# tasoc/photometry

Hardware: AMD Instinct MI355X
Metric: targets/sec (whole node), 10k targets x 1300 cad x 15x15, aperture + background (higher is better)
Workload: dtype f32

## Files before the change

### photometry_amd/csrc/aperture_dev.h

```cpp
#pragma once
#include "common.h"
#include <cmath>

namespace tp_ap {

constexpr int kMaxList = 128;
constexpr int kChunk = 1024;
constexpr int kMaxLeaves = 4096;
constexpr int kMaxDepth = 24;

template <int VEC> struct Vec;
template <> struct Vec<4> {
	static __device__ __forceinline__ void load(const float* p, float (&v)[4]) {
		float4 t = *reinterpret_cast<const float4*>(p);
		v[0] = t.x; v[1] = t.y; v[2] = t.z; v[3] = t.w;
	}
};
template <> struct Vec<2> {
	static __device__ __forceinline__ void load(const float* p, float (&v)[2]) {
		float2 t = *reinterpret_cast<const float2*>(p);
		v[0] = t.x; v[1] = t.y;
	}
};
template <> struct Vec<1> {
	static __device__ __forceinline__ void load(const float* p, float (&v)[1]) { v[0] = *p; }
};

template <int VEC>
struct CadState {
	float r[VEC][8];
	float e[VEC][8];
	float bk[VEC][8];
	float fres[VEC], eres[VEC], bres[VEC];
	double cw[VEC], ccol[VEC], crow[VEC];
	bool f_allnan[VEC], f_allzero[VEC], b_allnan[VEC];

	__device__ __forceinline__ void init() {
#pragma unroll
		for (int c = 0; c < VEC; c++) {
			fres[c] = 0.f; eres[c] = 0.f; bres[c] = 0.f;
			cw[c] = 0.0; ccol[c] = 0.0; crow[c] = 0.0;
			f_allnan[c] = true; f_allzero[c] = true; b_allnan[c] = true;
		}
	}
	__device__ __forceinline__ void side(const float (&v)[VEC], double col, double row) {
#pragma unroll
		for (int c = 0; c < VEC; c++) {
			const float x = v[c];
			f_allnan[c] = f_allnan[c] && (x != x);
			f_allzero[c] = f_allzero[c] && (x == 0.f);
			const double w = (x > 0.f) ? (double)x : 0.0;
			cw[c] += w;
			ccol[c] += col * w;
			crow[c] += row * w;
		}
	}
	__device__ __forceinline__ void bkg_terms(const float (&b)[VEC], float (&y)[VEC]) {
#pragma unroll
		for (int c = 0; c < VEC; c++) {
			const bool fin = (b[c] == b[c]);
			b_allnan[c] = b_allnan[c] && !fin;
			y[c] = fin ? b[c] : 0.f;
		}
	}
};

__device__ __forceinline__ float combine8(const float (&r)[8]) {
	return ((r[0] + r[1]) + (r[2] + r[3])) + ((r[4] + r[5]) + (r[6] + r[7]));
}

struct Args {
	const float* images; const float* images_err; const float* backgrounds;
	int32_t bkg_mode; int64_t bkg_series_pitch;
	const float* subtract; int64_t subtract_pitch;
	const uint8_t* mask; const int32_t* stamps; const int32_t* status;
	double* flux; double* flux_err; double* flux_bkg; double* ccol; double* crow;
	int64_t out_pitch; int n_cad; int height; int width; int64_t t_pitch; int n_targets;
	int32_t* big_list;
	int32_t stack_cols = 0, stack_row0 = 0, stack_col0 = 0;
};

__device__ __forceinline__ int64_t target_base(const Args& a, int target, int P) { return a.stack_cols ? 0 : (int64_t)target * P * a.t_pitch; }
__device__ __forceinline__ int stack_origin(const Args& a, int target) {
	return a.stack_cols ? ((a.stamps[target * 4 + 0] - a.stack_row0) * a.stack_cols + (a.stamps[target * 4 + 2] - a.stack_col0)) : 0;
}
__device__ __forceinline__ int pixel_row(const Args& a, int origin, int p, int pr, int pc) { return a.stack_cols ? (origin + pr * a.stack_cols + pc) : p; }

template <int VEC>
__device__ __forceinline__ void store_outputs(const Args& a, int target, int k0, const CadState<VEC>& st, int M) {
	const int64_t ob = (int64_t)target * a.out_pitch;
	const double nan = __builtin_nan("");
#pragma unroll
	for (int c = 0; c < VEC; c++) {
		const int k = k0 + c;
		if (k >= a.n_cad) continue;
		const bool bad = (M == 0) || st.f_allnan[c] || st.f_allzero[c];
		a.flux[ob + k] = bad ? nan : (double)st.fres[c];
		a.flux_err[ob + k] = bad ? nan : (double)sqrtf(st.eres[c]);
		const bool haspos = st.cw[c] > 0.0;
		a.ccol[ob + k] = (bad || !haspos) ? nan : st.ccol[c] / st.cw[c];
		a.crow[ob + k] = (bad || !haspos) ? nan : st.crow[c] / st.cw[c];
		if (a.flux_bkg) a.flux_bkg[ob + k] = (M == 0 || a.bkg_mode == 2 || st.b_allnan[c]) ? nan : (double)st.bres[c];
	}
}

__device__ __forceinline__ int compact_mask(const uint8_t* m, int P, int& p_next, int* list, int cap, int lane,
	bool count_rest, int* total)
{
	int n = 0;
	int p0 = p_next;
	for (; p0 < P; p0 += 64) {
		const int p = p0 + lane;
		const bool in = (p < P) && (m[p] != 0);
		const unsigned long long bal = __ballot(in);
		const int pos = n + __popcll(bal & ((1ull << lane) - 1ull));
		const int cnt = __popcll(bal);
		if (n + cnt > cap) {
			if (!count_rest) {
				if (in && pos < cap) list[pos] = p;
				const unsigned long long notstored = __ballot(in && pos >= cap);
				p_next = p0 + (int)__ffsll((long long)notstored) - 1;
				return cap;
			}
			if (in && pos < cap) list[pos] = p;
			n += cnt;
			continue;
		}
		if (in && pos < cap) list[pos] = p;
		n += cnt;
	}
	p_next = P;
	if (total) *total = n;
	return n < cap ? n : cap;
}

__device__ __forceinline__ void pack_rows(int* list, int M, int width, int lane, int nlanes) {
	for (int i = lane; i < M; i += nlanes) { const int p = list[i]; list[i] = p | ((p / width) << 16); }
}

template <int VEC>
__device__ __forceinline__ void extract_small(const Args& a, int target, const int* s_list, int M, int q_first, int q_stride)
{
	const int P = a.height * a.width;
	const int col0 = a.stamps[target * 4 + 2] + 1;
	const int row0 = a.stamps[target * 4 + 0] + 1;
	const int64_t tb = target_base(a, target, P);
	const int origin = stack_origin(a, target);
	const float* img = a.images + tb;
	const float* err = a.images_err + tb;
	const float* bkg = (a.bkg_mode == 0) ? (a.backgrounds + tb) : (a.backgrounds + (int64_t)target * a.bkg_series_pitch);
	const bool has_bkg = (a.bkg_mode != 2);
	const int nq = (a.n_cad + VEC - 1) / VEC;
	const int nblk = M - (M & 7);

	for (int q = q_first; q < nq; q += q_stride) {
		const int k0 = q * VEC;
		CadState<VEC> st;
		st.init();
		float bser[VEC], ssub[VEC];
		if (a.bkg_mode == 1) Vec<VEC>::load(bkg + k0, bser);
		if (a.subtract) Vec<VEC>::load(a.subtract + (int64_t)target * a.subtract_pitch + k0, ssub);

		auto fetch = [&](int idx, float (&v)[VEC], float (&e2)[VEC], float (&y)[VEC]) {
			const int pk = s_list[idx];
			const int p = pk & 0xffff;
			const int pr = (int)((unsigned)pk >> 16);
			const int pc = p - pr * a.width;
			const int64_t off = (int64_t)pixel_row(a, origin, p, pr, pc) * a.t_pitch + k0;
			float ee[VEC], bb[VEC];
			Vec<VEC>::load(img + off, v);
			if (a.subtract) {
#pragma unroll
				for (int c = 0; c < VEC; c++) v[c] = v[c] - ssub[c];
			}
			Vec<VEC>::load(err + off, ee);
			if (a.bkg_mode == 0) Vec<VEC>::load(bkg + off, bb);
			else {
#pragma unroll
				for (int c = 0; c < VEC; c++) bb[c] = (a.bkg_mode == 1) ? bser[c] : 0.f;
			}
#pragma unroll
			for (int c = 0; c < VEC; c++) e2[c] = ee[c] * ee[c];
			st.side(v, (double)(col0 + pc), (double)(row0 + pr));
			if (has_bkg) st.bkg_terms(bb, y);
		};

		if (M < 8) {
			for (int i = 0; i < M; i++) {
				float v[VEC], e2[VEC], y[VEC];
				fetch(i, v, e2, y);
#pragma unroll
				for (int c = 0; c < VEC; c++) { st.fres[c] += v[c]; st.eres[c] += e2[c]; if (has_bkg) st.bres[c] += y[c]; }
			}
		} else {
			for (int g = 0; g < nblk; g += 8) {
#pragma unroll
				for (int j = 0; j < 8; j++) {
					float v[VEC], e2[VEC], y[VEC];
					fetch(g + j, v, e2, y);
#pragma unroll
					for (int c = 0; c < VEC; c++) {
						if (g == 0) { st.r[c][j] = v[c]; st.e[c][j] = e2[c]; if (has_bkg) st.bk[c][j] = y[c]; }
						else { st.r[c][j] += v[c]; st.e[c][j] += e2[c]; if (has_bkg) st.bk[c][j] += y[c]; }
					}
				}
			}
#pragma unroll
			for (int c = 0; c < VEC; c++) { st.fres[c] = combine8(st.r[c]); st.eres[c] = combine8(st.e[c]); if (has_bkg) st.bres[c] = combine8(st.bk[c]); }
			for (int i = nblk; i < M; i++) {
				float v[VEC], e2[VEC], y[VEC];
				fetch(i, v, e2, y);
#pragma unroll
				for (int c = 0; c < VEC; c++) { st.fres[c] += v[c]; st.eres[c] += e2[c]; if (has_bkg) st.bres[c] += y[c]; }
			}
		}
#pragma unroll
		for (int c = 0; c < VEC; c++) { st.fres[c] = 0.f + st.fres[c]; st.eres[c] = 0.f + st.eres[c]; st.bres[c] = 0.f + st.bres[c]; }
		store_outputs<VEC>(a, target, k0, st, M);
	}
}

template <int VEC, bool HAS_SUB, int BKG, bool LDS_SERIES = false>
__device__ __forceinline__ void extract_small_stream(const Args& a, int target, const int* s_list, int M, int q_lane, int q_stride,
	const float* lds_sub = nullptr, const float* lds_ser = nullptr)
{
	const int P = a.height * a.width;
	const int col0 = a.stamps[target * 4 + 2] + 1;
	const int row0 = a.stamps[target * 4 + 0] + 1;
	const int64_t tb = (int64_t)target * P * a.t_pitch;
	const float* img = a.images + tb;
	const float* err = a.images_err + tb;
	constexpr bool BKG_CUBE = (BKG == 0), BKG_SERIES = (BKG == 1), HAS_BKG = (BKG != 2);
	const float* bkg = BKG_CUBE ? (a.backgrounds + tb) : (a.backgrounds + (int64_t)target * a.bkg_series_pitch);
	const float* subp = HAS_SUB ? (a.subtract + (int64_t)target * a.subtract_pitch) : nullptr;
	const int nq = (a.n_cad + VEC - 1) / VEC;
	const int nit = (nq + q_stride - 1) / q_stride;
	CadState<VEC> st;
	st.init();
	if (M == 0) {
		for (int it = 0; it < nit; it++) {
			const int q = q_lane + it * q_stride;
			if (q < nq) store_outputs<VEC>(a, target, q * VEC, st, 0);
		}
		return;
	}
	const int nfull = M >> 3, ntail = M & 7;
	const int spq = nfull + (ntail ? 1 : 0);
	const int total = nit * spq;

	struct Buf { float v[8][VEC], e[8][VEC], b[BKG_CUBE ? 8 : 1][VEC], ser[VEC], sub[VEC]; };
	Buf bufA, bufB;
	auto issue = [&](Buf& B, int step) {
		step = (step < total) ? step : (total - 1);
		const int it = step / spq, g = step - it * spq;
		int q = q_lane + it * q_stride;
		q = (q < nq) ? q : (nq - 1);
		const int k0 = q * VEC;
		if (BKG_SERIES) { if (LDS_SERIES) Vec<VEC>::load(lds_ser + k0, B.ser); else Vec<VEC>::load(bkg + k0, B.ser); }
		if (HAS_SUB) { if (LDS_SERIES) Vec<VEC>::load(lds_sub + k0, B.sub); else Vec<VEC>::load(subp + k0, B.sub); }
#pragma unroll
		for (int j = 0; j < 8; j++) {
			int idx = g * 8 + j;
			idx = (idx < M) ? idx : (M - 1);
			const int64_t rowoff = (int64_t)(__builtin_amdgcn_readfirstlane(s_list[idx]) & 0xffff) * a.t_pitch;
			Vec<VEC>::load(img + rowoff + k0, B.v[j]);
			Vec<VEC>::load(err + rowoff + k0, B.e[j]);
			if (BKG_CUBE) Vec<VEC>::load(bkg + rowoff + k0, B.b[j]);
		}
	};
	auto consume = [&](const Buf& B, int step) {
		if (step >= total) return;
		const int it = step / spq, g = step - it * spq;
		const int q = q_lane + it * q_stride;
		const bool full = g < nfull;
		const int cnt = full ? 8 : ntail;
#pragma unroll
		for (int j = 0; j < 8; j++) {
			if (j < cnt) {
				const int pk = __builtin_amdgcn_readfirstlane(s_list[g * 8 + j]);
				const int p = pk & 0xffff;
				const int pr = (int)((unsigned)pk >> 16);
				const int pc = p - pr * a.width;
				float v[VEC], e2[VEC], bb[VEC], y[VEC];
#pragma unroll
				for (int c = 0; c < VEC; c++) {
					v[c] = HAS_SUB ? (B.v[j][c] - B.sub[c]) : B.v[j][c];
					e2[c] = B.e[j][c] * B.e[j][c];
					bb[c] = BKG_CUBE ? B.b[BKG_CUBE ? j : 0][c] : (BKG_SERIES ? B.ser[c] : 0.f);
				}
				st.side(v, (double)(col0 + pc), (double)(row0 + pr));
				if (HAS_BKG) st.bkg_terms(bb, y);
#pragma unroll
				for (int c = 0; c < VEC; c++) {
					if (full) {
						if (g == 0) { st.r[c][j] = v[c]; st.e[c][j] = e2[c]; if (HAS_BKG) st.bk[c][j] = y[c]; }
						else { st.r[c][j] += v[c]; st.e[c][j] += e2[c]; if (HAS_BKG) st.bk[c][j] += y[c]; }
					} else { st.fres[c] += v[c]; st.eres[c] += e2[c]; if (HAS_BKG) st.bres[c] += y[c]; }
				}
			}
		}
		if (full && g == nfull - 1) {
#pragma unroll
			for (int c = 0; c < VEC; c++) { st.fres[c] = combine8(st.r[c]); st.eres[c] = combine8(st.e[c]); if (HAS_BKG) st.bres[c] = combine8(st.bk[c]); }
		}
		if (g == spq - 1) {
#pragma unroll
			for (int c = 0; c < VEC; c++) { st.fres[c] = 0.f + st.fres[c]; st.eres[c] = 0.f + st.eres[c]; st.bres[c] = 0.f + st.bres[c]; }
			if (q < nq) store_outputs<VEC>(a, target, q * VEC, st, M);
			st.init();
		}
	};
	issue(bufA, 0);
	issue(bufB, 1);
	for (int step = 0; step < total; step += 2) {
		consume(bufA, step);
		issue(bufA, step + 2);
		consume(bufB, step + 1);
		issue(bufB, step + 3);
	}
}

}

int tp_aperture_extract_big(tp_ctx* ctx, const tp_ap::Args& a, bool vec4);

void* tp_ctx_scratch(tp_ctx* ctx, size_t bytes);
```

### photometry_amd/csrc/fused.hip

```cpp
#include "sumimage_dev.h"
#include "aperture_dev.h"
#include "k2p2_args.h"
#include <algorithm>
#include <vector>

namespace {

constexpr int kRows = 8;

template <int VEC, bool VEC4, bool HAS_SUB, int BKG, bool A1>
__global__ __launch_bounds__(64, 2) void tp_aperture_fused_kernel(tp_ap::Args a, k2p2::BatchArgs ka, k2p2::Params prm,
	const double* __restrict__ twid, const int32_t* __restrict__ quality, int64_t quality_stride, uint32_t bitmask,
	double* __restrict__ sumimage_out, const int32_t* __restrict__ order)
{
	extern __shared__ __align__(16) unsigned char smem[];
	const int target = order ? order[blockIdx.x] : (int)blockIdx.x;
	const int lane = threadIdx.x;
	k2p2::Shared k;
	k2p2::shared_carve(k, smem, ka.H, ka.W, lane, twid);
	const int P = ka.H * ka.W;

	if constexpr (!A1) {
		const double* in = sumimage_out + (int64_t)target * P;
		for (int p = lane; p < P; p += 64) k.S[p] = in[p];
	} else {
	unsigned char* good = reinterpret_cast<unsigned char*>(k.srt);
	tp_sum::stage_good(good, quality + (int64_t)target * quality_stride, bitmask, a.n_cad, lane, 64);
	__syncthreads();
	{
		const float* base = a.images + (int64_t)target * P * a.t_pitch;
		const float* sub = a.subtract ? (a.subtract + (int64_t)target * a.subtract_pitch) : nullptr;
		double* o = sumimage_out + (int64_t)target * P;
		int p = 0;
		if (VEC4) {
			const int nq = ((a.n_cad + 3) & ~3) >> 2;
			const int spg = (nq + 63) >> 6;
			const int ngroups = (P + kRows - 1) / kRows;
			const uint32_t* good4 = reinterpret_cast<const uint32_t*>(good);
			const float4* sub4 = reinterpret_cast<const float4*>(sub);
			const float4 zero4 = make_float4(0.f, 0.f, 0.f, 0.f);
			const int total = ngroups * spg;
			float4 bufA[kRows], bufB[kRows];
			float4 subA = zero4, subB = zero4;
			auto issue = [&](float4 (&buf)[kRows], float4& sbuf, int st) {
				st = (st < total) ? st : (total - 1);
				const int g = st / spg, i = st - g * spg;
				int qd = lane + (i << 6);
				qd = (qd < nq) ? qd : (nq - 1);
				if (HAS_SUB) sbuf = sub4[qd];
#pragma unroll
				for (int j = 0; j < kRows; j++) {
					int r = g * kRows + j;
					r = (r < P) ? r : (P - 1);
					buf[j] = reinterpret_cast<const float4*>(base + (int64_t)r * a.t_pitch)[qd];
				}
			};
			double sacc[kRows];
			int nacc[kRows];
#pragma unroll
			for (int j = 0; j < kRows; j++) { sacc[j] = 0.0; nacc[j] = 0; }
			auto consume = [&](const float4 (&buf)[kRows], const float4& sa, int st) {
				const bool valid = st < total;
				const int g = st / spg, i = st - g * spg;
				const int qd = lane + (i << 6);
				if (valid && qd < nq) {
					const uint32_t gd = good4[qd];
#pragma unroll
					for (int j = 0; j < kRows; j++) {
						float4 v = buf[j];
						if (HAS_SUB) { v.x -= sa.x; v.y -= sa.y; v.z -= sa.z; v.w -= sa.w; }
						tp_sum::acc1(v.x, gd & 0xffu, sacc[j], nacc[j]); tp_sum::acc1(v.y, gd & 0xff00u, sacc[j], nacc[j]);
						tp_sum::acc1(v.z, gd & 0xff0000u, sacc[j], nacc[j]); tp_sum::acc1(v.w, gd & 0xff000000u, sacc[j], nacc[j]);
					}
				}
				if (valid && i == spg - 1) {
#pragma unroll
					for (int off = 32; off > 0; off >>= 1) {
#pragma unroll
						for (int j = 0; j < kRows; j++) { sacc[j] += __shfl_down(sacc[j], off, 64); nacc[j] += __shfl_down(nacc[j], off, 64); }
					}
					if (lane == 0) {
#pragma unroll
						for (int j = 0; j < kRows; j++) {
							const int r = g * kRows + j;
							if (r < P) { const double m = (nacc[j] > 0) ? sacc[j] / (double)nacc[j] : __builtin_nan(""); k.S[r] = m; o[r] = m; }
						}
					}
#pragma unroll
					for (int j = 0; j < kRows; j++) { sacc[j] = 0.0; nacc[j] = 0; }
				}
			};
			issue(bufA, subA, 0);
			issue(bufB, subB, 1);
			for (int st = 0; st < total; st += 2) {
				consume(bufA, subA, st);
				issue(bufA, subA, st + 2);
				consume(bufB, subB, st + 1);
				issue(bufB, subB, st + 3);
			}
		} else {
			for (; p < P; p++) {
				const double m = tp_sum::row_mean_scalar(base + (int64_t)p * a.t_pitch, sub, good, a.n_cad, lane);
				if (lane == 0) { k.S[p] = m; o[p] = m; }
			}
		}
	}
	}
	__syncthreads();

	k2p2::Target t;
	k2p2::make_target(ka, target, t);
	t.S = k.S;
	const int status = k2p2::run_target(k, prm, t);
	if (status == TP_STATUS_ERROR) return;

	int* s_list = reinterpret_cast<int*>(k.lab);
	int pn = 0, M = 0;
	tp_ap::compact_mask(k.res, P, pn, s_list, tp_ap::kMaxList, lane, true, &M);
	__syncthreads();
	if (M > tp_ap::kMaxList) {
		if (lane == 0 && a.big_list) a.big_list[1 + atomicAdd(&a.big_list[0], 1)] = target;
		return;
	}
	tp_ap::pack_rows(s_list, M, a.width, lane, 64);
	__syncthreads();
	const float* lds_sub = nullptr;
	const float* lds_ser = nullptr;
	{
		constexpr bool SER = (BKG == 1);
		const float* gsub = HAS_SUB ? (a.subtract + (int64_t)target * a.subtract_pitch) : nullptr;
		const float* gser = SER ? (a.backgrounds + (int64_t)target * a.bkg_series_pitch) : nullptr;
		const int nflt = (a.n_cad + VEC - 1) / VEC * VEC;
		const int room = (int)((reinterpret_cast<unsigned char*>(s_list) - smem) / sizeof(float));
		float* stage = reinterpret_cast<float*>(smem);
		const bool same = HAS_SUB && SER && (gsub == gser);
		const int need = ((HAS_SUB ? 1 : 0) + ((SER && !same) ? 1 : 0)) * nflt;
		if ((HAS_SUB || SER) && need > 0 && need <= room) {
			if (HAS_SUB) { for (int i = lane; i < nflt; i += 64) stage[i] = gsub[(i < a.n_cad) ? i : (a.n_cad - 1)]; lds_sub = stage; }
			if (SER) {
				if (same) lds_ser = stage;
				else { float* st2 = stage + (HAS_SUB ? nflt : 0); for (int i = lane; i < nflt; i += 64) st2[i] = gser[(i < a.n_cad) ? i : (a.n_cad - 1)]; lds_ser = st2; }
			}
			__syncthreads();
		}
	}
	if ((HAS_SUB && lds_sub) || (BKG == 1 && lds_ser)) tp_ap::extract_small_stream<VEC, HAS_SUB, BKG, true>(a, target, s_list, M, lane, 64, lds_sub, lds_ser);
	else tp_ap::extract_small_stream<VEC, HAS_SUB, BKG, false>(a, target, s_list, M, lane, 64);
}

}

static const int32_t* fused_launch_order(tp_ctx* ctx, const double* d_tmag, int n)
{
	if (n < 4096 || d_tmag == nullptr) return nullptr;
	if (ctx->order && ctx->order_key == (const void*)d_tmag && ctx->order_n == n) return ctx->order;
	std::vector<double> tm((size_t)n);
	if (hipMemcpyAsync(tm.data(), d_tmag, (size_t)n * sizeof(double), hipMemcpyDeviceToHost, ctx->stream) != hipSuccess) return nullptr;
	if (hipStreamSynchronize(ctx->stream) != hipSuccess) return nullptr;
	std::vector<int32_t> idx((size_t)n);
	for (int i = 0; i < n; ++i) idx[(size_t)i] = i;
	std::stable_sort(idx.begin(), idx.end(), [&](int32_t x, int32_t y) { return tm[(size_t)x] < tm[(size_t)y]; });
	if (ctx->order_n < n) {
		if (ctx->order) (void)hipFree(ctx->order);
		ctx->order = nullptr; ctx->order_n = 0;
		void* p = nullptr;
		if (tp_device_alloc(ctx, &p, (size_t)n * sizeof(int32_t)) != hipSuccess) return nullptr;
		ctx->order = static_cast<int32_t*>(p);
	}
	if (hipMemcpy(ctx->order, idx.data(), (size_t)n * sizeof(int32_t), hipMemcpyHostToDevice) != hipSuccess) { ctx->order_key = nullptr; return nullptr; }
	ctx->order_key = d_tmag; ctx->order_n = n;
	return ctx->order;
}

static int aperture_photometry_impl(tp_ctx* ctx, const tp_cube_desc* desc, bool given_sumimage,
	const float* d_images, const float* d_images_err, const float* d_backgrounds, int32_t bkg_mode, int64_t bkg_series_pitch,
	const float* d_subtract, int64_t subtract_pitch,
	const int32_t* d_quality, int64_t quality_target_stride, uint32_t bitmask,
	const int64_t* d_cat_offsets, const float* d_cat_column_stamp, const float* d_cat_row_stamp, const float* d_cat_tmag,
	const float* d_cat_column, const float* d_cat_row, const int64_t* d_cat_starid,
	const double* d_target_pos_row, const double* d_target_pos_column, const double* d_target_tmag, const int64_t* d_target_starid,
	const int32_t* d_stamps, const int32_t* d_aperture, const tp_k2p2_params* params,
	double* d_sumimage, uint8_t* d_mask, int32_t* d_status, int32_t* d_flags, double* d_contamination, double* d_diag,
	uint8_t* d_cat_in_mask,
	double* d_flux, double* d_flux_err, double* d_flux_background, double* d_centroid_col, double* d_centroid_row, int64_t out_pitch)
{
	TP_CHECK_CTX(ctx);
	TP_API_BEGIN
	TP_REQUIRE(ctx, tp_desc_ok(desc), "tp_aperture_photometry: bad cube descriptor");
	TP_REQUIRE(ctx, d_images && d_images_err && (d_quality || given_sumimage) && d_stamps && d_aperture && d_cat_offsets
		&& d_target_pos_row && d_target_pos_column && d_target_tmag && d_target_starid, "tp_aperture_photometry: null input pointer");
	TP_REQUIRE(ctx, d_sumimage && d_mask && d_status && d_flags && d_contamination, "tp_aperture_photometry: null output pointer");
	TP_REQUIRE(ctx, d_flux && d_flux_err && d_centroid_col && d_centroid_row, "tp_aperture_photometry: null output pointer");
	TP_REQUIRE(ctx, d_flux_background || !d_backgrounds, "tp_aperture_photometry: backgrounds given but no flux_background output");
	TP_REQUIRE(ctx, out_pitch >= desc->n_cad, "tp_aperture_photometry: out_pitch < n_cad");
	TP_REQUIRE(ctx, bkg_mode == 0 || bkg_mode == 1, "tp_aperture_photometry: bkg_mode must be 0 (cube) or 1 (series)");
	if (!d_backgrounds) bkg_mode = 2;
	TP_REQUIRE(ctx, bkg_mode != 1 || bkg_series_pitch >= desc->n_cad, "tp_aperture_photometry: bad bkg_series_pitch");
	TP_REQUIRE(ctx, quality_target_stride == 0 || quality_target_stride >= desc->n_cad, "tp_aperture_photometry: bad quality stride");
	TP_REQUIRE(ctx, d_subtract == nullptr || subtract_pitch >= desc->n_cad, "tp_aperture_photometry: bad subtract pitch");
	if (desc->n_targets == 0) return TP_OK;
	const int P = desc->height * desc->width;
	const k2p2::SharedLayout lay = k2p2::shared_layout(P);
	size_t shmem = lay.total;
	const size_t a1_bytes = lay.off_region + (size_t)((desc->n_cad + 3) & ~3) + 16;
	if (!given_sumimage && a1_bytes > shmem) shmem = a1_bytes;
	if (shmem > 160 * 1024) {
		int rc = given_sumimage ? TP_OK : tp_sumimage(ctx, desc, d_images, d_quality, quality_target_stride, bitmask, d_subtract, subtract_pitch, d_sumimage);
		if (rc != TP_OK) return rc;
		rc = tp_k2p2_masks(ctx, desc->n_targets, desc->height, desc->width, d_sumimage, d_cat_offsets, d_cat_column_stamp, d_cat_row_stamp,
			d_cat_tmag, d_cat_column, d_cat_row, d_cat_starid, d_target_pos_row, d_target_pos_column, d_target_tmag, d_target_starid,
			d_stamps, d_aperture, nullptr, params, d_mask, d_status, d_flags, d_contamination, d_diag, d_cat_in_mask);
		if (rc != TP_OK) return rc;
		return tp_aperture_extract(ctx, desc, d_images, d_images_err, d_backgrounds, (bkg_mode == 2) ? 0 : bkg_mode, bkg_series_pitch,
			d_subtract, subtract_pitch, d_mask, d_stamps, d_status, d_flux, d_flux_err, d_flux_background, d_centroid_col, d_centroid_row, out_pitch);
	}

	if (!ctx->twiddle) {
		double h[2 * k2p2::kGrid];
		for (int j = 0; j < k2p2::kGrid; ++j) {
			h[j] = std::cos(2.0 * k2p2::kPi * (double)j / (double)k2p2::kGrid);
			h[k2p2::kGrid + j] = std::sin(2.0 * k2p2::kPi * (double)j / (double)k2p2::kGrid);
		}
		TP_HIP(ctx, hipMalloc(&ctx->twiddle, sizeof(h)));
		TP_HIP(ctx, hipMemcpy(ctx->twiddle, h, sizeof(h), hipMemcpyHostToDevice));
	}

	k2p2::Params prm = k2p2::default_params();
	if (params) {
		prm.thresh = params->thresh;
		prm.min_no_pixels_in_mask = params->min_no_pixels_in_mask;
		prm.min_for_cluster = params->min_for_cluster;
		prm.extend_overflow = params->extend_overflow;
		prm.ws_thres = params->ws_thres;
		prm.saturation_limit = params->saturation_limit;
	}
	k2p2::BatchArgs ka;
	ka.n_targets = desc->n_targets; ka.H = desc->height; ka.W = desc->width; ka.sumimage = d_sumimage; ka.cat_offsets = d_cat_offsets;
	ka.cat_column_stamp = d_cat_column_stamp; ka.cat_row_stamp = d_cat_row_stamp; ka.cat_tmag = d_cat_tmag;
	ka.cat_column = d_cat_column; ka.cat_row = d_cat_row; ka.cat_starid = d_cat_starid;
	ka.target_pos_row = d_target_pos_row; ka.target_pos_column = d_target_pos_column; ka.target_tmag = d_target_tmag;
	ka.target_starid = d_target_starid; ka.stamps = d_stamps; ka.aperture = d_aperture; ka.cut_override = nullptr;
	ka.mask = d_mask; ka.status = d_status; ka.flags = d_flags; ka.contamination = d_contamination; ka.diag = d_diag;
	ka.cat_in_mask = d_cat_in_mask;

	tp_ap::Args a;
	a.images = d_images; a.images_err = d_images_err; a.backgrounds = d_backgrounds;
	a.bkg_mode = bkg_mode; a.bkg_series_pitch = bkg_series_pitch;
	a.subtract = d_subtract; a.subtract_pitch = subtract_pitch;
	a.mask = d_mask; a.stamps = d_stamps; a.status = d_status;
	a.flux = d_flux; a.flux_err = d_flux_err; a.flux_bkg = d_flux_background;
	a.ccol = d_centroid_col; a.crow = d_centroid_row;
	a.out_pitch = out_pitch; a.n_cad = desc->n_cad; a.height = desc->height; a.width = desc->width;
	a.t_pitch = desc->t_pitch; a.n_targets = desc->n_targets;
	a.big_list = static_cast<int32_t*>(tp_ctx_scratch(ctx, ((size_t)desc->n_targets + 1) * sizeof(int32_t)));
	TP_REQUIRE(ctx, a.big_list != nullptr, "tp_aperture_photometry: out of device memory for the work list");
	TP_HIP(ctx, hipMemsetAsync(a.big_list, 0, sizeof(int32_t), ctx->stream));

	bool vec4 = tp_vec4_ok(d_images, desc->t_pitch) && tp_vec4_ok(d_images_err, desc->t_pitch);
	if (bkg_mode == 0) vec4 = vec4 && tp_vec4_ok(d_backgrounds, desc->t_pitch);
	else if (bkg_mode == 1) vec4 = vec4 && tp_vec4_ok(d_backgrounds, bkg_series_pitch);
	if (d_subtract) vec4 = vec4 && tp_vec4_ok(d_subtract, subtract_pitch);

	const int32_t* d_order = fused_launch_order(ctx, d_target_tmag, desc->n_targets);
	const dim3 grid((unsigned)desc->n_targets), block(64);
#define TP_FUSED_LAUNCH_A(V, V4, HS, BK, A1) do { \
		auto kern = tp_aperture_fused_kernel<V, V4, HS, BK, A1>; \
		if (shmem > 64 * 1024) TP_HIP(ctx, hipFuncSetAttribute(reinterpret_cast<const void*>(kern), hipFuncAttributeMaxDynamicSharedMemorySize, (int)shmem)); \
		TP_LAUNCH(ctx, TPK_FUSED, kern, grid, block, shmem, a, ka, prm, (const double*)ctx->twiddle, d_quality, quality_target_stride, bitmask, d_sumimage, d_order); \
	} while (0)
#define TP_FUSED_LAUNCH(V, V4, HS, BK) do { if (given_sumimage) TP_FUSED_LAUNCH_A(V, V4, HS, BK, false); else TP_FUSED_LAUNCH_A(V, V4, HS, BK, true); } while (0)
#define TP_FUSED_BKG(V, V4, HS) do { \
		if (bkg_mode == 0) TP_FUSED_LAUNCH(V, V4, HS, 0); else if (bkg_mode == 1) TP_FUSED_LAUNCH(V, V4, HS, 1); else TP_FUSED_LAUNCH(V, V4, HS, 2); \
	} while (0)
	if (vec4) { if (d_subtract) TP_FUSED_BKG(2, true, true); else TP_FUSED_BKG(2, true, false); }
	else { if (d_subtract) TP_FUSED_BKG(1, false, true); else TP_FUSED_BKG(1, false, false); }
#undef TP_FUSED_BKG
#undef TP_FUSED_LAUNCH
#undef TP_FUSED_LAUNCH_A
	TP_LAUNCH_CHECK(ctx, "tp_aperture_fused_kernel");
	return tp_aperture_extract_big(ctx, a, vec4);
	TP_API_END(ctx)
}

extern "C" int tp_aperture_photometry(tp_ctx* ctx, const tp_cube_desc* desc,
	const float* d_images, const float* d_images_err, const float* d_backgrounds, int32_t bkg_mode, int64_t bkg_series_pitch,
	const float* d_subtract, int64_t subtract_pitch,
	const int32_t* d_quality, int64_t quality_target_stride, uint32_t bitmask,
	const int64_t* d_cat_offsets, const float* d_cat_column_stamp, const float* d_cat_row_stamp, const float* d_cat_tmag,
	const float* d_cat_column, const float* d_cat_row, const int64_t* d_cat_starid,
	const double* d_target_pos_row, const double* d_target_pos_column, const double* d_target_tmag, const int64_t* d_target_starid,
	const int32_t* d_stamps, const int32_t* d_aperture, const tp_k2p2_params* params,
	double* d_sumimage, uint8_t* d_mask, int32_t* d_status, int32_t* d_flags, double* d_contamination, double* d_diag,
	uint8_t* d_cat_in_mask,
	double* d_flux, double* d_flux_err, double* d_flux_background, double* d_centroid_col, double* d_centroid_row, int64_t out_pitch)
{
	return aperture_photometry_impl(ctx, desc, false, d_images, d_images_err, d_backgrounds, bkg_mode, bkg_series_pitch, d_subtract, subtract_pitch,
		d_quality, quality_target_stride, bitmask, d_cat_offsets, d_cat_column_stamp, d_cat_row_stamp, d_cat_tmag, d_cat_column, d_cat_row, d_cat_starid,
		d_target_pos_row, d_target_pos_column, d_target_tmag, d_target_starid, d_stamps, d_aperture, params, d_sumimage, d_mask, d_status, d_flags,
		d_contamination, d_diag, d_cat_in_mask, d_flux, d_flux_err, d_flux_background, d_centroid_col, d_centroid_row, out_pitch);
}

extern "C" int tp_aperture_photometry_from_sumimage(tp_ctx* ctx, const tp_cube_desc* desc,
	const float* d_images, const float* d_images_err, const float* d_backgrounds, int32_t bkg_mode, int64_t bkg_series_pitch,
	const float* d_subtract, int64_t subtract_pitch,
	const int32_t* d_quality, int64_t quality_target_stride, uint32_t bitmask,
	const int64_t* d_cat_offsets, const float* d_cat_column_stamp, const float* d_cat_row_stamp, const float* d_cat_tmag,
	const float* d_cat_column, const float* d_cat_row, const int64_t* d_cat_starid,
	const double* d_target_pos_row, const double* d_target_pos_column, const double* d_target_tmag, const int64_t* d_target_starid,
	const int32_t* d_stamps, const int32_t* d_aperture, const tp_k2p2_params* params,
	const double* d_sumimage, uint8_t* d_mask, int32_t* d_status, int32_t* d_flags, double* d_contamination, double* d_diag,
	uint8_t* d_cat_in_mask,
	double* d_flux, double* d_flux_err, double* d_flux_background, double* d_centroid_col, double* d_centroid_row, int64_t out_pitch)
{
	return aperture_photometry_impl(ctx, desc, true, d_images, d_images_err, d_backgrounds, bkg_mode, bkg_series_pitch, d_subtract, subtract_pitch,
		d_quality, quality_target_stride, bitmask, d_cat_offsets, d_cat_column_stamp, d_cat_row_stamp, d_cat_tmag, d_cat_column, d_cat_row, d_cat_starid,
		d_target_pos_row, d_target_pos_column, d_target_tmag, d_target_starid, d_stamps, d_aperture, params, const_cast<double*>(d_sumimage), d_mask, d_status, d_flags,
		d_contamination, d_diag, d_cat_in_mask, d_flux, d_flux_err, d_flux_background, d_centroid_col, d_centroid_row, out_pitch);
}
```

Before: 1.401 million.

## Precompute per-pixel offset and coordinate table in LDS for streaming aperture extraction

Builds a per-target LDS table of 32-bit byte offsets and double column/row coordinates, replacing per-pixel readfirstlane list decoding and 64-bit address math in the streaming loop. The step counters become incremental, which removes divisions. The accumulation is restructured with a new state struct that handles series backgrounds and optional FMA centroid accumulation. Launch bounds are raised to three waves per SIMD for most variants. It adds LDS usage, a fallback path when offsets overflow 32 bits, and may change rounding of centroid sums when FMA is used.

```diff
diff --git a/photometry_amd/csrc/aperture_dev.h b/photometry_amd/csrc/aperture_dev.h
--- a/photometry_amd/csrc/aperture_dev.h
+++ b/photometry_amd/csrc/aperture_dev.h
@@ -86,8 +86,8 @@
 }
 __device__ __forceinline__ int pixel_row(const Args& a, int origin, int p, int pr, int pc) { return a.stack_cols ? (origin + pr * a.stack_cols + pc) : p; }
 
-template <int VEC>
-__device__ __forceinline__ void store_outputs(const Args& a, int target, int k0, const CadState<VEC>& st, int M) {
+template <int VEC, class State>
+__device__ __forceinline__ void store_outputs(const Args& a, int target, int k0, const State& st, int M) {
 	const int64_t ob = (int64_t)target * a.out_pitch;
 	const double nan = __builtin_nan("");
 #pragma unroll
@@ -220,22 +220,78 @@
 	}
 }
 
-template <int VEC, bool HAS_SUB, int BKG, bool LDS_SERIES = false>
-__device__ __forceinline__ void extract_small_stream(const Args& a, int target, const int* s_list, int M, int q_lane, int q_stride,
+struct PixelTable { const double* col; const double* row; const uint32_t* off; };
+
+constexpr int kPixelEntryBytes = 20;
+__host__ __device__ inline int pixel_table_entries(int M) { return (M + 7) & ~7; }
+__host__ __device__ inline bool stream_offsets_fit(int64_t P, int64_t t_pitch) { return P * t_pitch * 4 < ((int64_t)1 << 32); }
+
+__device__ __forceinline__ PixelTable build_pixel_table(void* mem, const int* list, int M, const Args& a, int target, int lane, int nlanes)
+{
+	const int M8 = pixel_table_entries(M);
+	double* col = static_cast<double*>(mem);
+	double* row = col + M8;
+	uint32_t* off = reinterpret_cast<uint32_t*>(row + M8);
+	const int col0 = a.stamps[target * 4 + 2] + 1;
+	const int row0 = a.stamps[target * 4 + 0] + 1;
+	for (int i = lane; i < M8; i += nlanes) {
+		const int p = list[(i < M) ? i : (M - 1)];
+		const int pr = p / a.width, pc = p - pr * a.width;
+		off[i] = (uint32_t)p * (uint32_t)a.t_pitch * 4u;
+		col[i] = (double)(col0 + pc);
+		row[i] = (double)(row0 + pr);
+	}
+	PixelTable t;
+	t.col = col; t.row = row; t.off = off;
+	return t;
+}
+
+template <int VEC, int NBK>
+struct StreamState {
+	float r[VEC][8], e[VEC][8], bk[VEC][NBK];
+	float fres[VEC], eres[VEC], bres[VEC];
+	double cw[VEC], ccol[VEC], crow[VEC];
+	bool f_allnan[VEC], f_allzero[VEC], b_allnan[VEC];
+
+	__device__ __forceinline__ void init() {
+#pragma unroll
+		for (int c = 0; c < VEC; c++) {
+#pragma unroll
+			for (int j = 0; j < 8; j++) { r[c][j] = -0.f; e[c][j] = -0.f; }
+#pragma unroll
+			for (int j = 0; j < NBK; j++) bk[c][j] = -0.f;
+			fres[c] = 0.f; eres[c] = 0.f; bres[c] = 0.f;
+			cw[c] = 0.0; ccol[c] = 0.0; crow[c] = 0.0;
+			f_allnan[c] = true; f_allzero[c] = true; b_allnan[c] = true;
+		}
+	}
+	template <bool FUSE>
+	__device__ __forceinline__ void side(int c, float x, double col, double row) {
+		f_allnan[c] = f_allnan[c] && (x != x);
+		f_allzero[c] = f_allzero[c] && (x == 0.f);
+		const double w = (double)__builtin_fmaxf(x, 0.f);
+		cw[c] += w;
+		if (FUSE) { ccol[c] = __builtin_fma(col, w, ccol[c]); crow[c] = __builtin_fma(row, w, crow[c]); }
+		else { ccol[c] += col * w; crow[c] += row * w; }
+	}
+};
+
+#define TP_AP_KEEP_SCALAR(x) asm volatile("" : "+s"(x))
+template <int VEC, bool HAS_SUB, int BKG, bool LDS_SERIES, bool FUSE>
+__device__ __forceinline__ void extract_small_stream(const Args& a, int target, const PixelTable& tbl, int M, int q_lane, int q_stride,
 	const float* lds_sub = nullptr, const float* lds_ser = nullptr)
 {
 	const int P = a.height * a.width;
-	const int col0 = a.stamps[target * 4 + 2] + 1;
-	const int row0 = a.stamps[target * 4 + 0] + 1;
 	const int64_t tb = (int64_t)target * P * a.t_pitch;
-	const float* img = a.images + tb;
-	const float* err = a.images_err + tb;
 	constexpr bool BKG_CUBE = (BKG == 0), BKG_SERIES = (BKG == 1), HAS_BKG = (BKG != 2);
-	const float* bkg = BKG_CUBE ? (a.backgrounds + tb) : (a.backgrounds + (int64_t)target * a.bkg_series_pitch);
+	const char* img = reinterpret_cast<const char*>(a.images + tb);
+	const char* err = reinterpret_cast<const char*>(a.images_err + tb);
+	const char* bkgc = BKG_CUBE ? reinterpret_cast<const char*>(a.backgrounds + tb) : nullptr;
+	const float* bser = BKG_SERIES ? (a.backgrounds + (int64_t)target * a.bkg_series_pitch) : nullptr;
 	const float* subp = HAS_SUB ? (a.subtract + (int64_t)target * a.subtract_pitch) : nullptr;
 	const int nq = (a.n_cad + VEC - 1) / VEC;
 	const int nit = (nq + q_stride - 1) / q_stride;
-	CadState<VEC> st;
+	StreamState<VEC, BKG_CUBE ? 8 : 1> st;
 	st.init();
 	if (M == 0) {
 		for (int it = 0; it < nit; it++) {
@@ -246,79 +302,138 @@
 	}
 	const int nfull = M >> 3, ntail = M & 7;
 	const int spq = nfull + (ntail ? 1 : 0);
-	const int total = nit * spq;
 
 	struct Buf { float v[8][VEC], e[8][VEC], b[BKG_CUBE ? 8 : 1][VEC], ser[VEC], sub[VEC]; };
 	Buf bufA, bufB;
-	auto issue = [&](Buf& B, int step) {
-		step = (step < total) ? step : (total - 1);
-		const int it = step / spq, g = step - it * spq;
-		int q = q_lane + it * q_stride;
+	int it_i = 0, g_i = 0, it_c = 0, g_c = 0;
+	auto issue = [&](Buf& B) {
+		int q = q_lane + it_i * q_stride;
 		q = (q < nq) ? q : (nq - 1);
 		const int k0 = q * VEC;
-		if (BKG_SERIES) { if (LDS_SERIES) Vec<VEC>::load(lds_ser + k0, B.ser); else Vec<VEC>::load(bkg + k0, B.ser); }
-		if (HAS_SUB) { if (LDS_SERIES) Vec<VEC>::load(lds_sub + k0, B.sub); else Vec<VEC>::load(subp + k0, B.sub); }
+		if (!LDS_SERIES) {
+			if (BKG_SERIES) Vec<VEC>::load(bser + k0, B.ser);
+			if (HAS_SUB) Vec<VEC>::load(subp + k0, B.sub);
+		}
+		const uint4* to = reinterpret_cast<const uint4*>(tbl.off + g_i * 8);
+		const uint4 o0 = to[0], o1 = to[1];
+		const uint32_t ro[8] = { o0.x, o0.y, o0.z, o0.w, o1.x, o1.y, o1.z, o1.w };
+		const uint32_t kb = (uint32_t)k0 * 4u;
 #pragma unroll
 		for (int j = 0; j < 8; j++) {
-			int idx = g * 8 + j;
-			idx = (idx < M) ? idx : (M - 1);
-			const int64_t rowoff = (int64_t)(__builtin_amdgcn_readfirstlane(s_list[idx]) & 0xffff) * a.t_pitch;
-			Vec<VEC>::load(img + rowoff + k0, B.v[j]);
-			Vec<VEC>::load(err + rowoff + k0, B.e[j]);
-			if (BKG_CUBE) Vec<VEC>::load(bkg + rowoff + k0, B.b[j]);
-		}
+			const uint64_t vo = (uint64_t)(ro[j] + kb);
+			Vec<VEC>::load(reinterpret_cast<const float*>(img + vo), B.v[j]);
+			Vec<VEC>::load(reinterpret_cast<const float*>(err + vo), B.e[j]);
+			if (BKG_CUBE) Vec<VEC>::load(reinterpret_cast<const float*>(bkgc + vo), B.b[BKG_CUBE ? j : 0]);
+		}
+		if (++g_i == spq) { g_i = 0; ++it_i; }
+		if (it_i == nit) { it_i = nit - 1; g_i = spq - 1; }
 	};
-	auto consume = [&](const Buf& B, int step) {
-		if (step >= total) return;
-		const int it = step / spq, g = step - it * spq;
-		const int q = q_lane + it * q_stride;
-		const bool full = g < nfull;
-		const int cnt = full ? 8 : ntail;
-#pragma unroll
-		for (int j = 0; j < 8; j++) {
-			if (j < cnt) {
-				const int pk = __builtin_amdgcn_readfirstlane(s_list[g * 8 + j]);
-				const int p = pk & 0xffff;
-				const int pr = (int)((unsigned)pk >> 16);
-				const int pc = p - pr * a.width;
-				float v[VEC], e2[VEC], bb[VEC], y[VEC];
+	auto pixel = [&](const Buf& B, const float (&sub)[VEC], int j, double col, double row, float (&v)[VEC], float (&e2)[VEC], float (&y)[VEC]) {
+#pragma unroll
+		for (int c = 0; c < VEC; c++) {
+			v[c] = HAS_SUB ? (B.v[j][c] - sub[c]) : B.v[j][c];
+			e2[c] = B.e[j][c] * B.e[j][c];
+			st.template side<FUSE>(c, v[c], col, row);
+			if (BKG_CUBE) {
+				const float b = B.b[BKG_CUBE ? j : 0][c];
+				const bool fin = (b == b);
+				st.b_allnan[c] = st.b_allnan[c] && !fin;
+				y[c] = fin ? b : 0.f;
+			}
+		}
+	};
+	auto consume = [&](const Buf& B) {
+		if (it_c == nit) return;
+		const int q = q_lane + it_c * q_stride;
+		float ser[VEC], sub[VEC], yser[VEC];
+#pragma unroll
+		for (int c = 0; c < VEC; c++) { ser[c] = B.ser[c]; sub[c] = B.sub[c]; }
+		if (LDS_SERIES) {
+			const int k0 = ((q < nq) ? q : (nq - 1)) * VEC;
+			if (BKG_SERIES) Vec<VEC>::load(lds_ser + k0, ser);
+			if (HAS_SUB) Vec<VEC>::load(lds_sub + k0, sub);
+		}
+		if (BKG_SERIES) {
+#pragma unroll
+			for (int c = 0; c < VEC; c++) { const bool fin = (ser[c] == ser[c]); st.b_allnan[c] = !fin; yser[c] = fin ? ser[c] : 0.f; }
+		}
+		constexpr int NP = (LDS_SERIES && !BKG_CUBE) ? 4 : 2;
+		const double2* tc = reinterpret_cast<const double2*>(tbl.col + g_c * 8);
+		const double2* tr = reinterpret_cast<const double2*>(tbl.row + g_c * 8);
+		if (g_c < nfull) {
+#pragma unroll
+			for (int h = 0; h < 8 / NP; h++) {
+				if (h) __builtin_amdgcn_sched_barrier(0);
+				double col[NP], row[NP];
+#pragma unroll
+				for (int i = 0; i < NP / 2; i++) {
+					const double2 cc = tc[h * (NP / 2) + i], rr = tr[h * (NP / 2) + i];
+					col[2 * i] = cc.x; col[2 * i + 1] = cc.y; row[2 * i] = rr.x; row[2 * i + 1] = rr.y;
+				}
+#pragma unroll
+				for (int jj = 0; jj < NP; jj++) {
+					const int j = NP * h + jj;
+					float v[VEC], e2[VEC], y[VEC];
+					pixel(B, sub, j, col[jj], row[jj], v, e2, y);
+#pragma unroll
+					for (int c = 0; c < VEC; c++) { st.r[c][j] += v[c]; st.e[c][j] += e2[c]; if (BKG_CUBE) st.bk[c][BKG_CUBE ? j : 0] += y[c]; }
+				}
+			}
+			if (BKG_SERIES) {
+#pragma unroll
+				for (int c = 0; c < VEC; c++) st.bk[c][0] += yser[c];
+			}
+			if (g_c == nfull - 1) {
 #pragma unroll
 				for (int c = 0; c < VEC; c++) {
-					v[c] = HAS_SUB ? (B.v[j][c] - B.sub[c]) : B.v[j][c];
-					e2[c] = B.e[j][c] * B.e[j][c];
-					bb[c] = BKG_CUBE ? B.b[BKG_CUBE ? j : 0][c] : (BKG_SERIES ? B.ser[c] : 0.f);
+					st.r[c][0] = combine8(st.r[c]); st.e[c][0] = combine8(st.e[c]);
+					if constexpr (BKG_CUBE) st.bk[c][0] = combine8(st.bk[c]);
+					if constexpr (BKG_SERIES) { const float b = st.bk[c][0]; st.bk[c][0] = ((b + b) + (b + b)) + ((b + b) + (b + b)); }
 				}
-				st.side(v, (double)(col0 + pc), (double)(row0 + pr));
-				if (HAS_BKG) st.bkg_terms(bb, y);
-#pragma unroll
-				for (int c = 0; c < VEC; c++) {
-					if (full) {
-						if (g == 0) { st.r[c][j] = v[c]; st.e[c][j] = e2[c]; if (HAS_BKG) st.bk[c][j] = y[c]; }
-						else { st.r[c][j] += v[c]; st.e[c][j] += e2[c]; if (HAS_BKG) st.bk[c][j] += y[c]; }
-					} else { st.fres[c] += v[c]; st.eres[c] += e2[c]; if (HAS_BKG) st.bres[c] += y[c]; }
+			}
+		} else {
+			int cnt = ntail;
+			TP_AP_KEEP_SCALAR(cnt);
+#pragma unroll
+			for (int h = 0; h < 8 / NP; h++) {
+				if (NP * h < cnt) {
+					double col[NP], row[NP];
+#pragma unroll
+					for (int i = 0; i < NP / 2; i++) {
+						const double2 cc = tc[h * (NP / 2) + i], rr = tr[h * (NP / 2) + i];
+						col[2 * i] = cc.x; col[2 * i + 1] = cc.y; row[2 * i] = rr.x; row[2 * i + 1] = rr.y;
+					}
+#pragma unroll
+					for (int jj = 0; jj < NP; jj++) {
+						const int j = NP * h + jj;
+						if (j < cnt) {
+							float v[VEC], e2[VEC], y[VEC];
+							pixel(B, sub, j, col[jj], row[jj], v, e2, y);
+#pragma unroll
+							for (int c = 0; c < VEC; c++) { st.r[c][0] += v[c]; st.e[c][0] += e2[c]; if (HAS_BKG) st.bk[c][0] += BKG_SERIES ? yser[c] : y[c]; }
+						}
+					}
 				}
 			}
 		}
-		if (full && g == nfull - 1) {
-#pragma unroll
-			for (int c = 0; c < VEC; c++) { st.fres[c] = combine8(st.r[c]); st.eres[c] = combine8(st.e[c]); if (HAS_BKG) st.bres[c] = combine8(st.bk[c]); }
-		}
-		if (g == spq - 1) {
-#pragma unroll
-			for (int c = 0; c < VEC; c++) { st.fres[c] = 0.f + st.fres[c]; st.eres[c] = 0.f + st.eres[c]; st.bres[c] = 0.f + st.bres[c]; }
+		if (++g_c == spq) {
+#pragma unroll
+			for (int c = 0; c < VEC; c++) { st.fres[c] = 0.f + st.r[c][0]; st.eres[c] = 0.f + st.e[c][0]; st.bres[c] = HAS_BKG ? (0.f + st.bk[c][0]) : 0.f; }
 			if (q < nq) store_outputs<VEC>(a, target, q * VEC, st, M);
 			st.init();
+			g_c = 0; ++it_c;
 		}
 	};
-	issue(bufA, 0);
-	issue(bufB, 1);
-	for (int step = 0; step < total; step += 2) {
-		consume(bufA, step);
-		issue(bufA, step + 2);
-		consume(bufB, step + 1);
-		issue(bufB, step + 3);
-	}
-}
+	issue(bufA);
+	issue(bufB);
+	while (it_c < nit) {
+		consume(bufA);
+		issue(bufA);
+		consume(bufB);
+		issue(bufB);
+	}
+}
+#undef TP_AP_KEEP_SCALAR
 
 }
 
diff --git a/photometry_amd/csrc/fused.hip b/photometry_amd/csrc/fused.hip
--- a/photometry_amd/csrc/fused.hip
+++ b/photometry_amd/csrc/fused.hip
@@ -9,7 +9,7 @@
 constexpr int kRows = 8;
 
 template <int VEC, bool VEC4, bool HAS_SUB, int BKG, bool A1>
-__global__ __launch_bounds__(64, 2) void tp_aperture_fused_kernel(tp_ap::Args a, k2p2::BatchArgs ka, k2p2::Params prm,
+__global__ __launch_bounds__(64, (BKG == 0 && VEC == 2) ? 2 : 3) void tp_aperture_fused_kernel(tp_ap::Args a, k2p2::BatchArgs ka, k2p2::Params prm,
 	const double* __restrict__ twid, const int32_t* __restrict__ quality, int64_t quality_stride, uint32_t bitmask,
 	double* __restrict__ sumimage_out, const int32_t* __restrict__ order)
 {
@@ -122,7 +122,8 @@
 		if (lane == 0 && a.big_list) a.big_list[1 + atomicAdd(&a.big_list[0], 1)] = target;
 		return;
 	}
-	tp_ap::pack_rows(s_list, M, a.width, lane, 64);
+	const size_t table_bytes = (size_t)tp_ap::pixel_table_entries(M) * tp_ap::kPixelEntryBytes;
+	const tp_ap::PixelTable table = tp_ap::build_pixel_table(smem, s_list, M, a, target, lane, 64);
 	__syncthreads();
 	const float* lds_sub = nullptr;
 	const float* lds_ser = nullptr;
@@ -131,8 +132,8 @@
 		const float* gsub = HAS_SUB ? (a.subtract + (int64_t)target * a.subtract_pitch) : nullptr;
 		const float* gser = SER ? (a.backgrounds + (int64_t)target * a.bkg_series_pitch) : nullptr;
 		const int nflt = (a.n_cad + VEC - 1) / VEC * VEC;
-		const int room = (int)((reinterpret_cast<unsigned char*>(s_list) - smem) / sizeof(float));
-		float* stage = reinterpret_cast<float*>(smem);
+		const int room = (int)((reinterpret_cast<unsigned char*>(s_list) - (smem + table_bytes)) / sizeof(float));
+		float* stage = reinterpret_cast<float*>(smem + table_bytes);
 		const bool same = HAS_SUB && SER && (gsub == gser);
 		const int need = ((HAS_SUB ? 1 : 0) + ((SER && !same) ? 1 : 0)) * nflt;
 		if ((HAS_SUB || SER) && need > 0 && need <= room) {
@@ -144,8 +145,17 @@
 			__syncthreads();
 		}
 	}
-	if ((HAS_SUB && lds_sub) || (BKG == 1 && lds_ser)) tp_ap::extract_small_stream<VEC, HAS_SUB, BKG, true>(a, target, s_list, M, lane, 64, lds_sub, lds_ser);
-	else tp_ap::extract_small_stream<VEC, HAS_SUB, BKG, false>(a, target, s_list, M, lane, 64);
+	const int64_t cmax = (int64_t)std::abs((int64_t)a.stamps[target * 4 + 2] + 1) + a.width;
+	const int64_t rmax = (int64_t)std::abs((int64_t)a.stamps[target * 4 + 0] + 1) + a.height;
+	const bool fuse = cmax < ((int64_t)1 << 29) && rmax < ((int64_t)1 << 29);
+	const bool lds = (HAS_SUB && lds_sub) || (BKG == 1 && lds_ser);
+	if (lds) {
+		if (fuse) tp_ap::extract_small_stream<VEC, HAS_SUB, BKG, true, true>(a, target, table, M, lane, 64, lds_sub, lds_ser);
+		else tp_ap::extract_small_stream<VEC, HAS_SUB, BKG, true, false>(a, target, table, M, lane, 64, lds_sub, lds_ser);
+	} else {
+		if (fuse) tp_ap::extract_small_stream<VEC, HAS_SUB, BKG, false, true>(a, target, table, M, lane, 64);
+		else tp_ap::extract_small_stream<VEC, HAS_SUB, BKG, false, false>(a, target, table, M, lane, 64);
+	}
 }
 
 }
@@ -204,7 +214,7 @@
 	size_t shmem = lay.total;
 	const size_t a1_bytes = lay.off_region + (size_t)((desc->n_cad + 3) & ~3) + 16;
 	if (!given_sumimage && a1_bytes > shmem) shmem = a1_bytes;
-	if (shmem > 160 * 1024) {
+	if (shmem > 160 * 1024 || !tp_ap::stream_offsets_fit(P, desc->t_pitch)) {
 		int rc = given_sumimage ? TP_OK : tp_sumimage(ctx, desc, d_images, d_quality, quality_target_stride, bitmask, d_subtract, subtract_pitch, d_sumimage);
 		if (rc != TP_OK) return rc;
 		rc = tp_k2p2_masks(ctx, desc->n_targets, desc->height, desc->width, d_sumimage, d_cat_offsets, d_cat_column_stamp, d_cat_row_stamp,
```

Result: faster. 1.442 million, median of 6 (+2.9%).
